# bifurcationkit/BifurcationKit.jl

Measured on NVIDIA H100. Metric: continuation steps/sec (SH2d PALC), higher is better.
Workload: dtype f64

## Files before the change

bifurcationkit.jl_b200/csrc/bk_async.cuh:

```cuda
#pragma once
#include "bk_common.cuh"

#ifdef __CUDACC__
__device__ __forceinline__ unsigned bk2_smem(const void* p) { return (unsigned)__cvta_generic_to_shared(p); }
__device__ __forceinline__ void mbar_init(unsigned long long* b, unsigned cnt) {
  asm volatile("mbarrier.init.shared::cta.b64 [%0], %1;" ::"r"(bk2_smem(b)), "r"(cnt) : "memory");
}
__device__ __forceinline__ void mbar_arrive_expect_tx(unsigned long long* b, unsigned bytes) {
  asm volatile("mbarrier.arrive.expect_tx.shared::cta.b64 _, [%0], %1;" ::"r"(bk2_smem(b)), "r"(bytes) : "memory");
}
__device__ __forceinline__ void mbar_arrive(unsigned long long* b) {
  asm volatile("mbarrier.arrive.shared::cta.b64 _, [%0];" ::"r"(bk2_smem(b)) : "memory");
}
__device__ __forceinline__ void mbar_wait(unsigned long long* b, unsigned parity) {
  asm volatile(
      "{\n"
      ".reg .pred p;\n"
      "BK2_WAIT_%=:\n"
      "mbarrier.try_wait.parity.shared::cta.b64 p, [%0], %1;\n"
      "@p bra BK2_DONE_%=;\n"
      "bra BK2_WAIT_%=;\n"
      "BK2_DONE_%=:\n"
      "}\n" ::"r"(bk2_smem(b)),
      "r"(parity)
      : "memory");
}
__device__ __forceinline__ void bulk_g2s(void* dst, const void* src, unsigned bytes, unsigned long long* bar) {
  asm volatile("cp.async.bulk.shared::cluster.global.mbarrier::complete_tx::bytes [%0], [%1], %2, [%3];" ::"r"(bk2_smem(dst)),
               "l"(src), "r"(bytes), "r"(bk2_smem(bar))
               : "memory");
}
__device__ __forceinline__ void bulk_s2g(void* dst, const void* src, unsigned bytes) {
  asm volatile("cp.async.bulk.global.shared::cta.bulk_group [%0], [%1], %2;" ::"l"(dst), "r"(bk2_smem(src)), "r"(bytes) : "memory");
}
__device__ __forceinline__ void bulk_store_commit() { asm volatile("cp.async.bulk.commit_group;" ::: "memory"); }
__device__ __forceinline__ void bulk_store_wait_read() { asm volatile("cp.async.bulk.wait_group.read 0;" ::: "memory"); }
__device__ __forceinline__ void bulk_store_wait_all() { asm volatile("cp.async.bulk.wait_group 0;" ::: "memory"); }
__device__ __forceinline__ void bulk_prefetch_l2(const void* src, unsigned bytes) {
  asm volatile("cp.async.bulk.prefetch.L2.global [%0], %1;" ::"l"(src), "r"(bytes) : "memory");
}
__device__ __forceinline__ void fence_proxy_async_smem() { asm volatile("fence.proxy.async.shared::cta;" ::: "memory"); }
#ifndef BK2_NO_WAR_FENCE
__device__ __forceinline__ void consumer_release_fence() { asm volatile("fence.proxy.async.shared::cta;" ::: "memory"); }
#else
__device__ __forceinline__ void consumer_release_fence() {}
#endif
__device__ __forceinline__ void fence_mbar_init() { asm volatile("fence.mbarrier_init.release.cluster;" ::: "memory"); }

#endif
```

bifurcationkit.jl_b200/csrc/bk_common.cuh:

```cuda
#pragma once
#include <cuda_runtime.h>
#include <stdint.h>
#include <stdlib.h>
#include <string>
#include <unordered_map>
#include <vector>
#include "../../include/bk200.h"
#include <nvtx3/nvToolsExt.h>

struct BkRange {
  explicit BkRange(const char* name) { nvtxRangePushA(name); }
  ~BkRange() { nvtxRangePop(); }
};

#define BK_MAX_PAR 8
#define BK_NSM_FALLBACK 132

struct OpDesc {
  int kind;
  int nx, ny, nz;
  double cx, cy, cz;
  double par[BK_MAX_PAR];
  const double* u;
  double a0, a1;
// ... 26 lines not shown
}

enum { PW_NONE = 0, PW_RESID = 1, PW_JVP = 2, PW_FLEFT = 3, PW_FRIGHT = 4 };
struct PerPw {
  int pro;
  int epi;
  const double* v;
  const double* u;
  const double* sp;
  double a0, a1, l, nu;
  double spc;
};
#define PW_D 1

struct Precond {
  int kind = BK_PC_NONE;
  double a0 = 0, a1 = 0;
  double* lam[3] = {nullptr, nullptr, nullptr};
  int ttype[3] = {0, 0, 0};
  int fast[3] = {0, 0, 0};
  double2* ftw[3] = {nullptr, nullptr, nullptr};
  double2* fom[3] = {nullptr, nullptr, nullptr};
  double2* flam2[3] = {nullptr, nullptr, nullptr};
  bkg::Plan gplan[3] = {};
  double2* gwl[3] = {nullptr, nullptr, nullptr};
  double2* gph[3] = {nullptr, nullptr, nullptr};
  double* work = nullptr;
  double* work2 = nullptr;
  double* tri = nullptr;
  double2* tdft = nullptr;
  double po_r = 0, po_nu = 0, po_T = 0;
};

struct BkKindTraits {
  int ndims;
  int fields;
  int extra;
  bool jac_sym;
  bool has_jt;
  bool complex_ok;
  bool pow2_grid;
  bool has_jets;
};
const BkKindTraits* bk_kind_traits(int kind);

struct BkEventTimer {
  std::vector<std::pair<cudaEvent_t, cudaEvent_t>> pairs;
  size_t used = 0;
  void begin(cudaStream_t st) {
    if (used == pairs.size()) {
      cudaEvent_t a, b;
      cudaEventCreate(&a);
      cudaEventCreate(&b);
      pairs.push_back({a, b});
    }
    cudaEventRecord(pairs[used++].first, st);
  }
  void end(cudaStream_t st) { cudaEventRecord(pairs[used - 1].second, st); }
  long long harvest(double& ms) {
    long long k = 0;
    for (size_t i = 0; i < used; ++i) {
      float t = 0;
      if (cudaEventElapsedTime(&t, pairs[i].first, pairs[i].second) == cudaSuccess) {
        ms += t;
        ++k;
      }
    }
    used = 0;
    return k;
  }
  void destroy() {
    for (auto& p : pairs) {
      cudaEventDestroy(p.first);
      cudaEventDestroy(p.second);
    }
    pairs.clear();
    used = 0;
  }
};

struct bk_ctx {
  int device = 0;
  int nsm = BK_NSM_FALLBACK;
  cudaStream_t stream = nullptr;
  int kind = 0;
  long long dims[3] = {1, 1, 1};
  double lengths[3] = {1, 1, 1};
  double par[BK_MAX_PAR] = {0};
  long long N = 0;
  long long N0 = 0;
  bool cplx = false;
  double shift_imag = 0;
  bool transpose = false;
  int m = 0;
  long long ld = 0;
  double* u_state = nullptr;
  double jpar[BK_MAX_PAR] = {0};
  bool have_state = false;
  double* phi = nullptr;
  double* xpi = nullptr;
  double* fcache = nullptr;
  double phi_dot_xpi = 0;
  double* V = nullptr;
  double* w = nullptr;
  double* z = nullptr;
  double* r = nullptr;
  double* scales = nullptr;
  double* gcoef = nullptr;
  double* hcols = nullptr;
  double* hcols2 = nullptr;
  double* h_pinned = nullptr;
  double* partials = nullptr;
  int gmax = 0;
  unsigned int* counters = nullptr;
  double* red_out = nullptr;
  double* red_pinned = nullptr;
  double* coef_pinned = nullptr;
  std::vector<cudaEvent_t> events;
  std::vector<double*> stage;
  double* host_pinned = nullptr;
  std::vector<double*> tmp;
  double* mom_stage = nullptr;
  size_t mom_stage_cap = 0;
  void* mom_work = nullptr;
  size_t mom_work_cap = 0;
  double* defl_pinned = nullptr;
  std::unordered_map<double*, size_t> vec_live;
  std::vector<std::pair<size_t, double*>> vec_pool;
  double* Q = nullptr;
  double* Q2 = nullptr;
  int q2cap = 0;
  int qcap = 0;
  double* eig_dev = nullptr;
  double* eig_pinned = nullptr;
  Precond pc;
  bk_stats stats = {};
  bool timing = false;
  int timing_every = 1;
  long long solve_count = 0;
  bool timing_now = false;
  BkEventTimer fused_timer;
  BkEventTimer pc_timer;
  std::unordered_map<const void*, size_t> smem_attr;
  std::string err;
};

int bk_fail(bk_ctx* c, int code, const char* what, const char* file, int line);
#define BK_CUDA(c, expr)                                                             \
  do {                                                                               \
    cudaError_t _e = (expr);                                                         \
    if (_e != cudaSuccess) return bk_fail((c), BK_ERR_CUDA, cudaGetErrorString(_e), __FILE__, __LINE__); \
  } while (0)
#define BK_CHECK(c, cond, msg)                                                       \
  do {                                                                               \
    if (!(cond)) return bk_fail((c), BK_ERR_ARG, (msg), __FILE__, __LINE__);         \
  } while (0)
#define BK_ENTER(c)                                 \
  do {                                              \
    if (!(c)) return BK_ERR_ARG;                    \
    if (cudaSetDevice((c)->device) != cudaSuccess)  \
      return bk_fail((c), BK_ERR_CUDA, "cudaSetDevice failed", __FILE__, __LINE__); \
  } while (0)
#define BK_TRY(expr)                 \
  do {                               \
    int _s = (expr);                 \
    if (_s < 0) return _s;           \
// ... 166 lines not shown
```

bifurcationkit.jl_b200/csrc/bk_ctx.cu:

```cuda
#include <cstdio>
#include <cstring>
#include <map>
#include <mutex>
#include <new>
#include "bk_common.cuh"

int bk_fail(bk_ctx* c, int code, const char* what, const char* file, int line) {
  if (c) {
    char buf[512];
    snprintf(buf, sizeof buf, "%s (%s:%d)", what, file, line);
    c->err = buf;
  }
  return code;
}

void bk_grant_smem(int device, const void* kern, size_t bytes) {
  static std::mutex mu;
  static std::map<std::pair<int, const void*>, size_t> granted;
  std::lock_guard<std::mutex> lk(mu);
  size_t& cur = granted[{device, kern}];
  if (bytes <= cur) return;
  cudaFuncSetAttribute(kern, cudaFuncAttributeMaxDynamicSharedMemorySize, (int)bytes);
  if (bytes > 48 * 1024) cudaFuncSetAttribute(kern, cudaFuncAttributePreferredSharedMemoryCarveout, 100);
  cur = bytes;
// ... 13 lines not shown
  BK_CHECK(c, p != nullptr, "null vector argument");
  if (bk_is_device_ptr(p)) {
    *dev = const_cast<double*>(p);
    return BK_OK;
  }
  BK_CHECK(c, slot >= 0 && slot < 16, "bad stage slot");
  if ((int)c->stage.size() <= slot) c->stage.resize(slot + 1, nullptr);
  if (!c->stage[slot]) BK_CUDA(c, cudaMalloc(&c->stage[slot], sizeof(double) * (size_t)c->ld));
  BK_CHECK(c, n <= c->ld, "vector longer than the context's leading dimension");
  if (copy_in) {
    BK_CUDA(c, cudaMemcpyAsync(c->stage[slot], p, sizeof(double) * (size_t)n, cudaMemcpyHostToDevice, c->stream));
    c->stats.h2d_bytes += 8 * n;
  }
  *dev = c->stage[slot];
  return BK_OK;
}

int bk_stage_out(bk_ctx* c, double* p, long long n, const double* dev) {
  if (p == dev) return BK_OK;
  BK_CUDA(c, cudaMemcpyAsync(p, dev, sizeof(double) * (size_t)n, cudaMemcpyDeviceToHost, c->stream));
  BK_CUDA(c, cudaStreamSynchronize(c->stream));
  c->stats.d2h_bytes += 8 * n;
  return BK_OK;
}

int bk_tmp(bk_ctx* c, int slot, double** out) {
  if ((int)c->tmp.size() <= slot) c->tmp.resize(slot + 1, nullptr);
  if (!c->tmp[slot]) BK_CUDA(c, cudaMalloc(&c->tmp[slot], sizeof(double) * (size_t)c->ld));
  *out = c->tmp[slot];
  return BK_OK;
}

const BkKindTraits* bk_kind_traits(int kind) {
  static const BkKindTraits table[] = {{0, 0, 0, false, false, false, false, false},
                                       {1, 1, 0, false, false, true, false, true},
                                       {2, 1, 0, true, true, true, false, true},
                                       {3, 1, 0, true, true, true, false, true},
                                       {2, 2, 0, false, true, true, false, true},
                                       {3, 2, 1, false, true, false, false, false},
                                       {2, 1, 0, true, true, true, true, true}};
  static_assert(BK_CHAN == 1 && BK_POTRAP_CGL2D == 5 && BK_SH2D_PERIODIC == 6, "the table is indexed by kind");
  if (kind < BK_CHAN || kind > BK_SH2D_PERIODIC) return nullptr;
  return &table[kind];
}

extern "C" int32_t bk_ctx_create(int32_t device, int32_t kind, const int64_t dims[3], const double lengths[3],
                                 int32_t krylov_m, bk_ctx** out) {
  if (!out) return BK_ERR_ARG;
  *out = nullptr;
  bk_ctx* c = new (std::nothrow) bk_ctx();
  if (!c) return BK_ERR_ARG;
  *out = c;
  c->device = device;
  c->cplx = (kind & BK_COMPLEX) != 0;
  kind &= ~BK_COMPLEX;
  c->kind = kind;
  for (int i = 0; i < 3; ++i) {
    c->dims[i] = dims ? (dims[i] > 0 ? dims[i] : 1) : 1;
    c->lengths[i] = lengths ? lengths[i] : 1.0;
  }
  const BkKindTraits* kt = bk_kind_traits(kind);
  if (!kt) return bk_fail(c, BK_ERR_ARG, "unknown problem kind", __FILE__, __LINE__);
  if (kt->pow2_grid)
    for (int d = 0; d < 2; ++d) {
      const long long v = c->dims[d];
      BK_CHECK(c, v >= 64 && v <= 2048 && (v & (v - 1)) == 0,
               "BK_SH2D_PERIODIC: Nx and Ny must be powers of two from 64 to 2048");
    }
  long long n = kt->fields;
  for (int d = 0; d < kt->ndims; ++d) n *= c->dims[d];
  n += kt->extra;
  BK_CHECK(c, n >= 2, "problem too small");
  BK_CHECK(c, krylov_m >= 1 && krylov_m <= 1024, "krylov_m out of range");
  BK_CHECK(c, !c->cplx || kt->complex_ok, "BK_COMPLEX is not available for the periodic-orbit functional");
  c->N0 = n;
  if (c->cplx) n *= 2;
  c->N = n;
  c->m = krylov_m;
  c->ld = ((n + 2 + 31) / 32) * 32;
  BK_CUDA(c, cudaSetDevice(device));
  cudaDeviceProp prop;
  BK_CUDA(c, cudaGetDeviceProperties(&prop, device));
  c->nsm = prop.multiProcessorCount;
  if (const char* e = getenv("BK_NSM")) {
    const int v = atoi(e);
    if (v >= 1 && v <= 1024) c->nsm = v;
  }
  BK_CUDA(c, cudaStreamCreateWithFlags(&c->stream, cudaStreamNonBlocking));
  size_t ld = (size_t)c->ld, m = (size_t)c->m;
  BK_CUDA(c, cudaMalloc(&c->u_state, 8 * ld));
  BK_CUDA(c, cudaMalloc(&c->V, 8 * ld * (m + 1)));
  BK_CUDA(c, cudaMalloc(&c->w, 8 * ld));
  BK_CUDA(c, cudaMalloc(&c->z, 8 * ld));
  BK_CUDA(c, cudaMalloc(&c->r, 8 * ld));
  BK_CUDA(c, cudaMemset(c->u_state, 0, 8 * ld));
  BK_CUDA(c, cudaMemset(c->V, 0, 8 * ld * (m + 1)));
  BK_CUDA(c, cudaMemset(c->w, 0, 8 * ld));
  BK_CUDA(c, cudaMemset(c->z, 0, 8 * ld));
  BK_CUDA(c, cudaMemset(c->r, 0, 8 * ld));
  BK_CUDA(c, cudaMalloc(&c->scales, 8 * (m + 4)));
  BK_CUDA(c, cudaMalloc(&c->gcoef, 8 * (m + 4)));
  BK_CUDA(c, cudaMalloc(&c->hcols, 8 * (m + 1) * (m + 4)));
  BK_CUDA(c, cudaMalloc(&c->hcols2, 8 * (m + 1) * (m + 4)));
  BK_CUDA(c, cudaMemset(c->hcols, 0, 8 * (m + 1) * (m + 4)));
  BK_CUDA(c, cudaMemset(c->hcols2, 0, 8 * (m + 1) * (m + 4)));
  BK_CUDA(c, cudaMallocHost(&c->h_pinned, 2 * 8 * (m + 1) * (m + 4)));
  long long g = (n + 2 + 255) / 256 + 8;
  if (kind == BK_SH2D) {
    long long gf = ((c->dims[0] + 255) / 256) * c->dims[1] + 8;
    if (gf > g) g = gf;
  }
  if (g < 4 * c->nsm) g = 4 * c->nsm;
  c->gmax = (int)g;
  BK_CUDA(c, cudaMalloc(&c->partials, 8 * (m + 4) * (size_t)c->gmax));
  BK_CUDA(c, cudaMalloc(&c->counters, 64 * sizeof(unsigned int)));
  BK_CUDA(c, cudaMemset(c->counters, 0, 64 * sizeof(unsigned int)));
  BK_CUDA(c, cudaMalloc(&c->red_out, 8 * 16));
  BK_CUDA(c, cudaMallocHost(&c->red_pinned, 8 * 16));
  BK_CUDA(c, cudaMallocHost(&c->coef_pinned, 8 * (m + 4)));
  c->events.resize(m + 2);
  for (auto& e : c->events) BK_CUDA(c, cudaEventCreateWithFlags(&e, cudaEventDisableTiming));
  if (kind == BK_POTRAP_CGL2D) {
    BK_CUDA(c, cudaMalloc(&c->phi, 8 * ld));
    BK_CUDA(c, cudaMalloc(&c->xpi, 8 * ld));
    BK_CUDA(c, cudaMalloc(&c->fcache, 8 * ld));
    BK_CUDA(c, cudaMemset(c->phi, 0, 8 * ld));
    BK_CUDA(c, cudaMemset(c->xpi, 0, 8 * ld));
  }
  if (kind == BK_SH2D_PERIODIC) BK_TRY(bk_periodic_setup(c));
  BK_CUDA(c, cudaStreamSynchronize(c->stream));
  return BK_OK;
}

extern "C" int32_t bk_ctx_destroy(bk_ctx* c) {
  if (!c) return BK_OK;
  cudaSetDevice(c->device);
  if (c->stream) cudaStreamSynchronize(c->stream);
  double* bufs[] = {c->u_state, c->V, c->w, c->z, c->r, c->scales, c->gcoef, c->hcols, c->hcols2, c->partials,
                    c->red_out, c->phi, c->xpi, c->fcache, c->pc.work, c->pc.work2, c->pc.tri, c->Q, c->Q2, c->eig_dev};
  for (double* b : bufs)
    if (b) cudaFree(b);
  for (int d = 0; d < 3; ++d) {
    void* tabs[] = {c->pc.lam[d], c->pc.ftw[d], c->pc.fom[d], c->pc.flam2[d], c->pc.gwl[d], c->pc.gph[d]};
    for (void* t : tabs)
      if (t) cudaFree(t);
  }
  if (c->pc.tdft) cudaFree(c->pc.tdft);
  if (c->counters) cudaFree(c->counters);
  for (auto& kv : c->vec_live) cudaFree(kv.first);
  for (double* b : c->stage)
    if (b) cudaFree(b);
  for (double* b : c->tmp)
    if (b) cudaFree(b);
  if (c->mom_stage) cudaFree(c->mom_stage);
  if (c->mom_work) cudaFree(c->mom_work);
  if (c->defl_pinned) cudaFreeHost(c->defl_pinned);
  if (c->h_pinned) cudaFreeHost(c->h_pinned);
  if (c->red_pinned) cudaFreeHost(c->red_pinned);
  if (c->coef_pinned) cudaFreeHost(c->coef_pinned);
  if (c->host_pinned) cudaFreeHost(c->host_pinned);
  if (c->eig_pinned) cudaFreeHost(c->eig_pinned);
  for (auto& e : c->events)
    if (e) cudaEventDestroy(e);
  c->fused_timer.destroy();
  c->pc_timer.destroy();
  if (c->stream) cudaStreamDestroy(c->stream);
// ... 214 lines not shown
```

bifurcationkit.jl_b200/csrc/bk_krylov.cu:

```cuda
#include <cmath>
#include <cstdlib>
#include <cstring>
#include <vector>
#include "bk_common.cuh"
#include "bk_stencil.cuh"
#include "bk_krylov_tma.cuh"

static __global__ void __launch_bounds__(BK_THREADS) k_lincomb(double* __restrict__ x, double beta, long long n,
                                                               const double* __restrict__ V, long long ld, int k,
                                                               const double* __restrict__ coef,
                                                               const double* __restrict__ scales) {
  const long long base = (long long)blockIdx.x * BK_TILE;
  double val[BK_EPT];
  int off[BK_EPT];
  bool ok[BK_EPT];
#pragma unroll
  for (int e = 0; e < BK_EPT; ++e) {
    long long g = base + threadIdx.x + e * BK_THREADS;
    ok[e] = g < n;
    off[e] = ok[e] ? (int)g : 0;
    val[e] = (ok[e] && beta != 0.0) ? beta * x[g] : 0.0;
  }
  for (int i = 0; i < k; ++i) {
    const double ci = coef[i] * (scales ? scales[i] : 1.0);
    const double* Vi = V + (long long)i * ld;
#pragma unroll
    for (int e = 0; e < BK_EPT; ++e) val[e] = fma(ci, __ldg(Vi + off[e]), val[e]);
  }
#pragma unroll
  for (int e = 0; e < BK_EPT; ++e)
    if (ok[e]) x[off[e]] = val[e];
}


#define BK2_BLOCKS_PER_SM 4
struct Plan2 {
  int E, grid, NS, sred_off;
  size_t smem;
};
static inline size_t bk2_budget() { return (size_t)(233472 / BK2_BLOCKS_PER_SM) - 1024 - 512; }

static Plan2 plan2(bk_ctx* c, long long units_of_256, size_t scratch_bytes_per_E(int), int force_E = 0) {
  Plan2 p;
  const long long slots = (long long)c->nsm * BK2_BLOCKS_PER_SM;
  long long E = BK2_EMAX;
  while (E > 1 && (units_of_256 + E - 1) / E < (17 * (long long)c->nsm) / 10) --E;
  if ((units_of_256 + E - 1) / E > slots) {
    double best = -1.0;
    for (long long cand = BK2_EMAX; cand >= 5; --cand) {
      long long g = (units_of_256 + cand - 1) / cand, w = (g + slots - 1) / slots;
      double eff = (double)g / (double)(w * slots);
      if (eff > best + 1e-9) {
        best = eff;
        E = cand;
      }
    }
  }
  if (force_E) E = force_E;
  {
    static const int env_e = [] {
      const char* a = getenv("BK2_E");
      return a ? atoi(a) : 0;
    }();
    if (env_e >= 1 && env_e <= BK2_EMAX) E = env_e;
  }
  p.E = (int)E;
  p.grid = (int)((units_of_256 + E - 1) / E);
  const size_t sred = sizeof(double) * 8 * (size_t)(c->m + 2);
  const size_t stage = sizeof(double) * (size_t)E * BK2_ROW;
  size_t budget = bk2_budget();
  long long ns = budget > sred ? (long long)((budget - sred) / stage) : 2;
  if (ns > BK2_MAXSTAGES) ns = BK2_MAXSTAGES;
  if (ns < 2) ns = 2;
  p.NS = (int)ns;
  size_t ring = stage * (size_t)p.NS;
  size_t scratch = scratch_bytes_per_E ? scratch_bytes_per_E(p.E) : 0;
  size_t lo = ring > scratch ? ring : scratch;
  lo = (lo + 127) / 128 * 128;
  p.sred_off = (int)(lo / sizeof(double));
  p.smem = lo + sred;
  return p;
}
static size_t sh2_scratch_bytes(int E) { return sizeof(double) * (size_t)((BK2_ROW + 4) * (E + 4) + (BK2_ROW + 2) * (E + 2)); }

#define BK2_DISPATCH(E, ...) \
  switch (E) {                \
    case 1: { constexpr int EE = 1; __VA_ARGS__; } break; \
    case 2: { constexpr int EE = 2; __VA_ARGS__; } break; \
    case 3: { constexpr int EE = 3; __VA_ARGS__; } break; \
    case 4: { constexpr int EE = 4; __VA_ARGS__; } break; \
    case 5: { constexpr int EE = 5; __VA_ARGS__; } break; \
    case 6: { constexpr int EE = 6; __VA_ARGS__; } break; \
    case 7: { constexpr int EE = 7; __VA_ARGS__; } break; \
    default: { constexpr int EE = 8; __VA_ARGS__; } break; \
  }

static bool fuses_jvp(const bk_ctx* c, const OpDesc& op, const bk_gmres_opts* o) {
  const bool left = o->pc_side == BK_SIDE_LEFT && c->pc.kind != BK_PC_NONE;
  return o->fused && op.kind == BK_SH2D && op.nx % 2 == 0 && !op.cplx && op.bordered <= 1 && !left;
}

static bool fuses_pc(const bk_ctx* c, const OpDesc& op, const bk_gmres_opts* o) {
  const bool side = o->pc_side == BK_SIDE_LEFT || o->pc_side == BK_SIDE_RIGHT;
  return o->fused && op.kind == BK_SH2D_PERIODIC && c->pc.kind == BK_PC_SH_FFT && side && op.bordered == 0 && !op.cplx;
}

static int launch_fused(bk_ctx* c, const OpDesc& op, const double* in, const double* sp, double* w, int j, double* hcol) {
  const int tiles_x = (op.nx + BK2_ROW - 1) / BK2_ROW;
  Plan2 p = plan2(c, (long long)tiles_x * op.ny, sh2_scratch_bytes);
  p.grid = tiles_x * ((op.ny + p.E - 1) / p.E);
  BK_CHECK(c, p.grid <= c->gmax, "partial-sum workspace too small for the fused grid");
  BK2_DISPATCH(p.E, {
    auto kern = op.bordered ? k2_fused<EE, true> : k2_fused<EE, false>;
    return bk_launch(c, kern, dim3(p.grid), dim3(BK2_THREADS), p.smem, op, in, sp, w, c->V, c->ld, j, c->scales, c->partials,
                     c->counters + 0, hcol, c->gcoef, p.NS, p.sred_off);
  });
}

static inline int chunk_grid(long long n) { return (int)((n + BK_TILE - 1) / BK_TILE); }

int bk_launch_dots(bk_ctx* c, const double* basis, const double* scales, const double* w, long long n, int j, double* hcol,
                   double* gcoef) {
  Plan2 p = plan2(c, (n + BK2_ROW - 1) / BK2_ROW, nullptr);
  BK_CHECK(c, p.grid <= c->gmax, "partial-sum workspace too small");
  BK2_DISPATCH(p.E, return bk_launch(c, k2_dots<EE>, dim3(p.grid), dim3(BK2_THREADS), p.smem, w, n, basis, c->ld, j, scales,
                                     c->partials, c->counters + 1, hcol, gcoef, p.NS, p.sred_off));
}
static int launch_dots(bk_ctx* c, const double* w, long long n, int j, double* hcol) {
  return bk_launch_dots(c, c->V, c->scales, w, n, j, hcol, c->gcoef);
}

int bk_launch_update(bk_ctx* c, const double* basis, const double* gcoef, const double* w, long long n, int j, double* vout,
                     double* h_out, double* scale_out) {
  Plan2 p = plan2(c, (n + BK2_ROW - 1) / BK2_ROW, nullptr);
  BK_CHECK(c, p.grid <= c->gmax, "partial-sum workspace too small");
  BK2_DISPATCH(p.E, return bk_launch(c, k2_update<EE>, dim3(p.grid), dim3(BK2_THREADS), p.smem, w, n, basis, c->ld, j, gcoef, vout,
                                     c->partials, c->counters + 2, h_out, scale_out, p.NS));
}
static int launch_update(bk_ctx* c, const double* w, long long n, int j, double* vout, double* h_out, double* scale_out) {
  return bk_launch_update(c, c->V, c->gcoef, w, n, j, vout, h_out, scale_out);
}

int bk_launch_lincomb(bk_ctx* c, const double* basis, const double* scales, double* x, double beta, long long n, int k,
                      const double* coef_dev) {
  return bk_launch_ordered(c, k_lincomb, chunk_grid(n), BK_THREADS, 0, x, beta, n, basis, c->ld, k, coef_dev, scales);
}
static int launch_lincomb(bk_ctx* c, double* x, double beta, long long n, int k, const double* coef_dev, bool use_scales) {
  return bk_launch_lincomb(c, c->V, use_scales ? c->scales : nullptr, x, beta, n, k, coef_dev);
}

static int arnoldi_step(bk_ctx* c, const OpDesc& op, const bk_gmres_opts* o, long long n, int k, bool fuse, bool fuse_pc) {
  const int j = k + 1;
  const int mh = c->m + 4;
  double* hcol = c->h_pinned + (size_t)k * mh;
  double* hcol2 = c->h_pinned + (size_t)(c->m + 1) * mh + (size_t)k * mh;
  const double* in = c->V + (size_t)k * c->ld;
  const double* sp = c->scales + k;
  const bool left = o->pc_side == BK_SIDE_LEFT && c->pc.kind != BK_PC_NONE;
  const bool right = o->pc_side == BK_SIDE_RIGHT && c->pc.kind != BK_PC_NONE;
  if (right && !fuse_pc) {
    BK_TRY(bk_precond_apply_dev(c, in, c->z, n));
    in = c->z;
  }
  const bool timed = c->timing_now;
  const double* wfin = c->w;
  if (fuse_pc) {
    BK_TRY(bk_periodic_fused(c, op, in, sp, c->w, left));
  } else if (!fuse) {
    BK_TRY(bk_launch_apply(c, op, in, sp, c->w));
    if (left) {
      BK_TRY(bk_precond_apply_dev(c, c->w, c->r, n));
      wfin = c->r;
    }
  }
  if (timed) c->fused_timer.begin(c->stream);
  BK_TRY(fuse ? launch_fused(c, op, in, sp, c->w, j, hcol) : launch_dots(c, wfin, n, j, hcol));
  if (timed) c->fused_timer.end(c->stream);
  double* vnext = c->V + (size_t)(k + 1) * c->ld;
  if (timed) c->fused_timer.begin(c->stream);
  BK_TRY(launch_update(c, wfin, n, j, vnext, hcol + j, c->scales + k + 1));
  if (timed) c->fused_timer.end(c->stream);
  if (o->orth == BK_ORTH_CGS2) {
    BK_TRY(launch_dots(c, vnext, n, j, hcol2));
    BK_TRY(launch_update(c, vnext, n, j, vnext, hcol + j, c->scales + k + 1));
  }
  BK_CUDA(c, cudaEventRecord(c->events[k], c->stream));
  const long long step_bytes = 8LL * n * (2LL * j + 4) + (op.bordered ? 16LL * n : 0LL);
  c->stats.last_fused_bytes += step_bytes;
  c->stats.last_fused_launches += 2;
  if (fuse && (c->timing_now || !c->timing)) {
    c->stats.total_fused_bytes += step_bytes;
    c->stats.total_fused_launches += 2;
  }
  return BK_OK;
}

static int init_residual(bk_ctx* c, const OpDesc& op, const bk_gmres_opts* o, long long n, const double* rhs, const double* x,
                         bool x_zero, double* beta) {
  const bool left = o->pc_side == BK_SIDE_LEFT && c->pc.kind != BK_PC_NONE;
  const double* r = rhs;
  if (!x_zero) {
    BK_TRY(bk_launch_apply(c, op, x, nullptr, c->w));
    BK_TRY(bk_dev_axpby(c, c->w, 1.0, rhs, -1.0, n));
    r = c->w;
  }
  if (left) {
    BK_TRY(bk_precond_apply_dev(c, r, c->r, n));
    r = c->r;
  }
  BK_TRY(launch_update(c, r, n, 0, c->V, c->red_out, c->scales));
  BK_CUDA(c, cudaMemcpyAsync(c->red_pinned, c->red_out, 8, cudaMemcpyDeviceToHost, c->stream));
  BK_CUDA(c, cudaStreamSynchronize(c->stream));
  *beta = c->red_pinned[0];
  return BK_OK;
}

int bk_gmres_dev(bk_ctx* c, const OpDesc& op, const double* rhs, double* x, const bk_gmres_opts* o, int* converged,
                 int* iters, double* resnorm) {
  const long long n = op.N + op.bordered;
  BK_CHECK(c, n <= c->ld, "system larger than the context");
// ... 183 lines not shown
```

bifurcationkit.jl_b200/csrc/bk_krylov_tma.cuh:

```cuda
#pragma once
#include "bk_common.cuh"
#include "bk_async.cuh"

#define BK2_CONS 256
#define BK2_THREADS 288
#define BK2_EMAX 8
#define BK2_ROW 256

struct Tile2 {
  long long base;
  int rs;
  int rows;
  int len;
  int last_len;
};

#define BK2_MAXSTAGES 8
struct Ring {
  unsigned long long full[BK2_MAXSTAGES];
  unsigned long long empty[BK2_MAXSTAGES];
};

__device__ __forceinline__ void ring_init(Ring* rg, int NS) {
  if (threadIdx.x == 0) {
    for (int s = 0; s < NS; ++s) {
      mbar_init(&rg->full[s], 1);
      mbar_init(&rg->empty[s], 8);
    }
    fence_mbar_init();
  }
}

template <int E, int MODE, bool REV = false>
__device__ __forceinline__ void stream_basis(const Tile2& tl, const double* __restrict__ V, long long ld, int j, double* ring,
                                             int NS, Ring* rg, double (&val)[E], double* sred,
                                             const double* __restrict__ gcoef) {
  const int warp = threadIdx.x >> 5, lane = threadIdx.x & 31;
  if (warp == 8) {
    if (lane == 0) {
      fence_proxy_async_smem();
      const unsigned row_b = (unsigned)(((tl.len + 1) & ~1) * 8);
      const unsigned last_b = (unsigned)(((tl.last_len + 1) & ~1) * 8);
      const bool contiguous = (tl.rs == BK2_ROW) && (tl.len == BK2_ROW);
      const unsigned total = row_b * (unsigned)(tl.rows - 1) + last_b;
      for (int i = 0; i < j; ++i) {
        const int s = i % NS, round = i / NS;
        if (round > 0) mbar_wait(&rg->empty[s], (unsigned)((round - 1) & 1));
        mbar_arrive_expect_tx(&rg->full[s], total);
        const double* src = V + (long long)(REV ? j - 1 - i : i) * ld + tl.base;
        double* dst = ring + (size_t)s * (E * BK2_ROW);
        if (contiguous) {
          bulk_g2s(dst, src, total, &rg->full[s]);
        } else {
          for (int r = 0; r < tl.rows - 1; ++r) bulk_g2s(dst + r * BK2_ROW, src + (long long)r * tl.rs, row_b, &rg->full[s]);
          bulk_g2s(dst + (tl.rows - 1) * BK2_ROW, src + (long long)(tl.rows - 1) * tl.rs, last_b, &rg->full[s]);
        }
      }
    }
  } else {
    const int t = threadIdx.x;
    if (MODE == 0) {
      for (int i = 0; i < j; i += 2) {
        const int s0 = i % NS, s1 = (i + 1) % NS;
        const bool two = (i + 1 < j);
        mbar_wait(&rg->full[s0], (unsigned)((i / NS) & 1));
        const double* st0 = ring + (size_t)s0 * (E * BK2_ROW) + t;
        double a0 = 0.0, a1 = 0.0;
#pragma unroll
        for (int e = 0; e < E; ++e) {
          const int lim = (e == tl.rows - 1) ? tl.last_len : tl.len;
          if (e < tl.rows && t < lim) a0 = fma(st0[e * BK2_ROW], val[e], a0);
        }
        if (two) {
          mbar_wait(&rg->full[s1], (unsigned)(((i + 1) / NS) & 1));
          const double* st1 = ring + (size_t)s1 * (E * BK2_ROW) + t;
#pragma unroll
          for (int e = 0; e < E; ++e) {
            const int lim = (e == tl.rows - 1) ? tl.last_len : tl.len;
            if (e < tl.rows && t < lim) a1 = fma(st1[e * BK2_ROW], val[e], a1);
          }
        }
        consumer_release_fence();
        __syncwarp();
        if (lane == 0) {
          mbar_arrive(&rg->empty[s0]);
          if (two) mbar_arrive(&rg->empty[s1]);
        }
#pragma unroll
        for (int o = 16; o > 0; o >>= 1) {
          a0 += __shfl_xor_sync(0xffffffffu, a0, o);
          a1 += __shfl_xor_sync(0xffffffffu, a1, o);
        }
        if (lane == 0) {
          sred[i * 8 + warp] = a0;
          if (two) sred[(i + 1) * 8 + warp] = a1;
        }
      }
    } else {
      for (int i = 0; i < j; ++i) {
        const int s = i % NS;
        mbar_wait(&rg->full[s], (unsigned)((i / NS) & 1));
        const double* st = ring + (size_t)s * (E * BK2_ROW) + t;
        const double g = __ldg(gcoef + (REV ? j - 1 - i : i));
#pragma unroll
        for (int e = 0; e < E; ++e) {
          const int lim = (e == tl.rows - 1) ? tl.last_len : tl.len;
          if (e < tl.rows && t < lim) val[e] = fma(-g, st[e * BK2_ROW], val[e]);
        }
        consumer_release_fence();
        __syncwarp();
        if (lane == 0) mbar_arrive(&rg->empty[s]);
      }
    }
  }
}

struct BorderFin {
  double bscale, bc, xp;
  double* w_tail;
  const double* V_tail;
  long long ld;
};
__device__ __forceinline__ void dots_finish(int j, const double* sred, const double* __restrict__ scales,
                                            double* __restrict__ partials, unsigned int* counter, double* __restrict__ hcol,
                                            double* __restrict__ gcoef, int* s_flag, const BorderFin* bord = nullptr,
                                            double* s_wp = nullptr) {
  const int G = gridDim.x;
  const int jj = bord ? j + 1 : j;
  for (int i = threadIdx.x; i < jj; i += blockDim.x) {
    double t = 0.0;
#pragma unroll
    for (int k = 0; k < 8; ++k) t += sred[i * 8 + k];
    partials[(long long)i * G + blockIdx.x] = t;
  }
  if (bk_last_block(counter, s_flag)) {
    const int warp = threadIdx.x >> 5, lane = threadIdx.x & 31, nw = blockDim.x >> 5;
    double wp = 0.0;
    if (bord) {
      if (warp == 0) {
        double t = 0.0;
        for (int k = lane; k < G; k += 32) t += __ldcg(partials + (long long)j * G + k);
        t = bk_warp_sum(t);
        if (lane == 0) {
          *s_wp = bord->bscale * t + bord->bc * bord->xp;
          *bord->w_tail = *s_wp;
        }
      }
      __syncthreads();
      wp = *s_wp;
    }
    for (int i = warp; i < j; i += nw) {
      double t = 0.0;
      for (int k = lane; k < G; k += 32) t += __ldcg(partials + (long long)i * G + k);
      t = bk_warp_sum(t);
      if (lane == 0) {
        if (bord) t = fma(__ldg(bord->V_tail + (long long)i * bord->ld), wp, t);
        const double s = scales[i];
        const double h = s * t;
        hcol[i] = h;
        gcoef[i] = h * s;
      }
    }
  }
}

template <int E>
struct Sh2Scratch {
  static constexpr int VX = BK2_ROW + 4, VY = E + 4, QX = BK2_ROW + 2, QY = E + 2;
  static constexpr int V_ELEMS = VX * VY, Q_ELEMS = QX * QY;
  static constexpr size_t BYTES = sizeof(double) * (size_t)(V_ELEMS + Q_ELEMS);
};

template <int E>
__device__ __forceinline__ void sh2_tile_issue(const OpDesc& op, const double* __restrict__ in, int x0, int y0, double* scratch,
                                               unsigned long long* tbar) {
  using S = Sh2Scratch<E>;
  const int nx = op.nx, ny = op.ny;
  const int len = min(BK2_ROW, nx - x0);
  mbar_arrive_expect_tx(tbar, (unsigned)(len * 8) * (unsigned)S::VY);
#pragma unroll 1
  for (int jj = 0; jj < S::VY; ++jj) {
    int gy = y0 - 2 + jj;
    gy = gy < 0 ? 0 : (gy > ny - 1 ? ny - 1 : gy);
    bulk_g2s(scratch + jj * S::VX + 2, in + x0 + (long long)gy * nx, (unsigned)(len * 8), tbar);
  }
}

template <int E, bool BORDERED, bool RESID = false>
__device__ __forceinline__ void sh2_tile_eval(const OpDesc& op, const double* __restrict__ in, double in_scale, int x0, int y0,
                                              double* scratch, unsigned long long* tbar, double (&val)[E], double xp,
                                              double* bsum) {
  using S = Sh2Scratch<E>;
  double* vs = scratch;
  double* qs = scratch + S::V_ELEMS;
  const int nx = op.nx, ny = op.ny;
  const int len = min(BK2_ROW, nx - x0);
  if (threadIdx.x < 4 * S::VY) {
    const int jj = threadIdx.x >> 2, h = threadIdx.x & 3;
    const int i = h < 2 ? h : len + h;
    int gx = x0 - 2 + i, gy = y0 - 2 + jj;
    gx = gx < 0 ? 0 : (gx > nx - 1 ? nx - 1 : gx);
    gy = gy < 0 ? 0 : (gy > ny - 1 ? ny - 1 : gy);
    vs[jj * S::VX + i] = __ldg(in + gx + (long long)gy * nx);
  }
  mbar_wait(tbar, 0);
  __syncthreads();
  for (int q = threadIdx.x; q < S::Q_ELEMS; q += blockDim.x) {
    int i = q % S::QX, jj = q / S::QX;
    int cx = x0 - 1 + i, cy = y0 - 1 + jj;
    cx = (cx < 0 ? 0 : (cx > nx - 1 ? nx - 1 : cx)) - (x0 - 2);
    cy = (cy < 0 ? 0 : (cy > ny - 1 ? ny - 1 : cy)) - (y0 - 2);
    const double* p = vs + cx + cy * S::VX;
    const double c0 = p[0];
    qs[q] = c0 + op.cx * (p[-1] - 2.0 * c0 + p[1]) + op.cy * (p[-S::VX] - 2.0 * c0 + p[S::VX]);
  }
  __syncthreads();
  const int t = threadIdx.x;
  const double l = op.par[0], nu = op.par[1];
  const int gx = x0 + t;
  const bool colok = t < BK2_ROW && gx < nx;
  const int rows = min(E, ny - y0);
  double g[E];
  if (!RESID) {
#pragma unroll
    for (int e = 0; e < E; ++e) g[e] = (colok && e < rows) ? __ldg(op.u + gx + (long long)(y0 + e) * nx) : 0.0;
  }
#pragma unroll
  for (int e = 0; e < E; ++e) {
    double r = 0.0;
    if (colok && e < rows) {
      const double* p = qs + (t + 1) + (e + 1) * S::QX;
      const double c0 = p[0];
      const double l1v = in_scale * (c0 + op.cx * (p[-1] - 2.0 * c0 + p[1]) + op.cy * (p[-S::QX] - 2.0 * c0 + p[S::QX]));
      const double v = in_scale * vs[(t + 2) + (e + 2) * S::VX];
      if (RESID) {
        r = v * (l + v * (nu - v)) - l1v;
      } else {
        const double coef = l + g[e] * (2.0 * nu - 3.0 * g[e]);
        r = op.a0 * v + op.a1 * (coef * v - l1v);
        if (BORDERED) r += op.bshift * v;
      }
    }
    val[e] = r;
  }
  if (BORDERED) {
#pragma unroll
    for (int e = 0; e < E; ++e) g[e] = (colok && e < rows) ? __ldg(op.ba + gx + (long long)(y0 + e) * nx) : 0.0;
#pragma unroll
    for (int e = 0; e < E; ++e) val[e] = fma(xp, g[e], val[e]);
#pragma unroll
    for (int e = 0; e < E; ++e) g[e] = (colok && e < rows) ? __ldg(op.bb + gx + (long long)(y0 + e) * nx) : 0.0;
#pragma unroll
    for (int e = 0; e < E; ++e)
      if (colok && e < rows) *bsum = fma(g[e], in_scale * vs[(t + 2) + (e + 2) * S::VX], *bsum);
  }
}

template <int E, bool BORDERED>
static __global__ void __launch_bounds__(BK2_THREADS, 4) k2_fused(OpDesc op, const double* __restrict__ in,
                                                                  const double* __restrict__ in_scale_ptr,
                                                                  double* __restrict__ w, const double* __restrict__ V,
                                                                  long long ld, int j, const double* __restrict__ scales,
                                                                  double* __restrict__ partials, unsigned int* counter,
                                                                  double* __restrict__ hcol, double* __restrict__ gcoef,
                                                                  int NS, int sred_off) {
  extern __shared__ __align__(128) double smem2[];
  __shared__ Ring rg;
  __shared__ __align__(8) unsigned long long tbar;
  __shared__ int s_flag;
  double* ring = smem2;
  double* sred = smem2 + sred_off;
  if (threadIdx.x == 0) mbar_init(&tbar, 1);
  ring_init(&rg, NS);
  const int tiles_x = (op.nx + BK2_ROW - 1) / BK2_ROW;
  const int x0 = (blockIdx.x % tiles_x) * BK2_ROW, y0 = (blockIdx.x / tiles_x) * E;
  double val[E];
  Tile2 tl;
  tl.base = x0 + (long long)y0 * op.nx;
  tl.rs = op.nx;
  tl.rows = min(E, op.ny - y0);
  tl.len = min(BK2_ROW, op.nx - x0);
  tl.last_len = tl.len;
  __syncthreads();
  bk_pdl_sync();
  const double s = in_scale_ptr ? __ldg(in_scale_ptr) : 1.0;
  if (threadIdx.x == BK2_CONS) {
    sh2_tile_issue<E>(op, in, x0, y0, smem2, &tbar);
    const unsigned row_b = (unsigned)(((tl.len + 1) & ~1) * 8);
    for (int r = 0; r < tl.rows; ++r) {
      const long long o = tl.base + (long long)r * tl.rs;
      bulk_prefetch_l2(op.u + o, row_b);
      if (BORDERED) {
        bulk_prefetch_l2(op.ba + o, row_b);
        bulk_prefetch_l2(op.bb + o, row_b);
      }
    }
    const int npf = j < 2 * NS ? j : 2 * NS;
    for (int i = 0; i < npf; ++i)
      for (int r = 0; r < tl.rows; ++r) bulk_prefetch_l2(V + (long long)i * ld + tl.base + (long long)r * tl.rs, row_b);
  }
  const double xp = BORDERED ? s * __ldg(in + op.N) : 0.0;
  double bsum = 0.0;
  sh2_tile_eval<E, BORDERED>(op, in, s, x0, y0, smem2, &tbar, val, xp, &bsum);
  if (threadIdx.x < tl.len) {
#pragma unroll
    for (int e = 0; e < E; ++e)
      if (e < tl.rows) w[tl.base + (long long)e * tl.rs + threadIdx.x] = val[e];
  }
  fence_proxy_async_smem();
  __syncthreads();
  stream_basis<E, 0>(tl, V, ld, j, ring, NS, &rg, val, sred, nullptr);
  if (BORDERED) {
    __shared__ double s_wp;
    bsum = bk_warp_sum(bsum);
    if ((threadIdx.x & 31) == 0 && threadIdx.x < BK2_CONS) sred[j * 8 + (threadIdx.x >> 5)] = bsum;
    __syncthreads();
    BorderFin bf;
    bf.bscale = op.bscale;
    bf.bc = op.bc;
    bf.xp = xp;
    bf.w_tail = w + op.N;
    bf.V_tail = V + op.N;
    bf.ld = ld;
    dots_finish(j, sred, scales, partials, counter, hcol, gcoef, &s_flag, &bf, &s_wp);
  } else {
    __syncthreads();
    dots_finish(j, sred, scales, partials, counter, hcol, gcoef, &s_flag);
  }
}

template <int E, int MODE>
static __global__ void __launch_bounds__(BK2_THREADS, 4) k2_apply(OpDesc op, const double* __restrict__ in,
                                                                  const double* __restrict__ in_scale_ptr, double* __restrict__ out) {
  extern __shared__ __align__(128) double smem2[];
  __shared__ __align__(8) unsigned long long tbar;
  if (threadIdx.x == 0) {
    mbar_init(&tbar, 1);
    fence_mbar_init();
  }
  const int tiles_x = (op.nx + BK2_ROW - 1) / BK2_ROW;
  const int x0 = (blockIdx.x % tiles_x) * BK2_ROW, y0 = (blockIdx.x / tiles_x) * E;
  const int rows = min(E, op.ny - y0), len = min(BK2_ROW, op.nx - x0);
  __syncthreads();
  const double s = in_scale_ptr ? __ldg(in_scale_ptr) : 1.0;
  if (threadIdx.x == BK2_CONS) {
    sh2_tile_issue<E>(op, in, x0, y0, smem2, &tbar);
    if (MODE == 0) {
      const unsigned row_b = (unsigned)(len * 8);
      for (int r = 0; r < rows; ++r) bulk_prefetch_l2(op.u + x0 + (long long)(y0 + r) * op.nx, row_b);
    }
  }
  double val[E];
  double bsum = 0.0;
  sh2_tile_eval<E, false, MODE == 1>(op, in, s, x0, y0, smem2, &tbar, val, 0.0, &bsum);
  if (threadIdx.x < len) {
#pragma unroll
    for (int e = 0; e < E; ++e)
      if (e < rows) out[x0 + (long long)(y0 + e) * op.nx + threadIdx.x] = val[e];
  }
}

__device__ __forceinline__ Tile2 linear_tile(long long n, int E) {
  Tile2 tl;
  tl.base = (long long)blockIdx.x * (E * BK2_ROW);
  tl.rs = BK2_ROW;
  long long rem = n - tl.base;
  int rows = (int)((rem + BK2_ROW - 1) / BK2_ROW);
  tl.rows = rows < E ? rows : E;
  tl.len = BK2_ROW;
  long long lastrem = rem - (long long)(tl.rows - 1) * BK2_ROW;
  tl.last_len = lastrem < BK2_ROW ? (int)lastrem : BK2_ROW;
  if (tl.rows == 1) tl.len = tl.last_len;
  return tl;
}

template <int E>
static __global__ void __launch_bounds__(BK2_THREADS, 4) k2_dots(const double* __restrict__ w, long long n,
                                                                 const double* __restrict__ V, long long ld, int j,
                                                                 const double* __restrict__ scales,
                                                                 double* __restrict__ partials, unsigned int* counter,
                                                                 double* __restrict__ hcol, double* __restrict__ gcoef, int NS,
                                                                 int sred_off) {
  extern __shared__ __align__(128) double smem2[];
  __shared__ Ring rg;
  __shared__ int s_flag;
  double* ring = smem2;
  double* sred = smem2 + sred_off;
  ring_init(&rg, NS);
  const Tile2 tl = linear_tile(n, E);
  double val[E];
  bk_pdl_sync();
#pragma unroll
  for (int e = 0; e < E; ++e) {
    const int lim = (e == tl.rows - 1) ? tl.last_len : tl.len;
    val[e] = (threadIdx.x < BK2_ROW && e < tl.rows && (int)threadIdx.x < lim) ? w[tl.base + e * BK2_ROW + threadIdx.x] : 0.0;
  }
  __syncthreads();
  stream_basis<E, 0>(tl, V, ld, j, ring, NS, &rg, val, sred, nullptr);
  __syncthreads();
  dots_finish(j, sred, scales, partials, counter, hcol, gcoef, &s_flag);
}

template <int E>
static __global__ void __launch_bounds__(BK2_THREADS, 4) k2_update(const double* w, long long n,
                                                                   const double* __restrict__ V, long long ld, int j,
                                                                   const double* __restrict__ gcoef, double* vout,
                                                                   double* __restrict__ partials, unsigned int* counter,
                                                                   double* __restrict__ h_out, double* __restrict__ scale_out,
                                                                   int NS) {
  extern __shared__ __align__(128) double smem2[];
  __shared__ Ring rg;
  __shared__ double s_w[9];
  __shared__ int s_flag;
  double* ring = smem2;
  ring_init(&rg, NS);
  const Tile2 tl = linear_tile(n, E);
  double val[E];
  const int t = threadIdx.x;
  bk_pdl_sync();
#pragma unroll
  for (int e = 0; e < E; ++e) {
    const int lim = (e == tl.rows - 1) ? tl.last_len : tl.len;
    val[e] = (t < BK2_ROW && e < tl.rows && t < lim) ? w[tl.base + e * BK2_ROW + t] : 0.0;
  }
  __syncthreads();
  stream_basis<E, 1, true>(tl, V, ld, j, ring, NS, &rg, val, nullptr, gcoef);
  double acc = 0.0;
  if (t < BK2_ROW) {
#pragma unroll
    for (int e = 0; e < E; ++e) {
      const int lim = (e == tl.rows - 1) ? tl.last_len : tl.len;
      if (e < tl.rows && t < lim) {
        vout[tl.base + e * BK2_ROW + t] = val[e];
        acc = fma(val[e], val[e], acc);
      }
    }
  }
  acc = bk_warp_sum(acc);
  const int lane = t & 31, wid = t >> 5;
  if (lane == 0) s_w[wid] = acc;
  __syncthreads();
  if (t == 0) {
    double r = 0;
    for (int k = 0; k < 9; ++k) r += s_w[k];
    partials[blockIdx.x] = r;
  }
  if (bk_last_block(counter, &s_flag)) {
    double r = 0.0;
    for (int k = t; k < (int)gridDim.x; k += blockDim.x) r += __ldcg(partials + k);
    r = bk_warp_sum(r);
    if (lane == 0) s_w[wid] = r;
    __syncthreads();
    if (t == 0) {
      double q = 0;
      for (int k = 0; k < 9; ++k) q += s_w[k];
      const double h = sqrt(q);
      *h_out = h;
      *scale_out = 1.0 / h;
    }
  }
}
```

Before: 4.343.

## Add L2 evict-first/evict-last hints to Krylov basis streaming and reorder fused kernel

Krylov basis loads through the bulk-copy ring now carry an L2 cache policy. The last `keep` vectors, sized to about half the L2, are marked evict-last so they stay resident for the next kernel; older ones are marked evict-first. The explicit L2 prefetch of the first basis vectors in the fused kernel is removed. The stencil kernel issues its state loads before the halo barrier, and the fused kernel writes w after streaming the basis rather than before. The aim is fewer DRAM re-reads of recently used basis vectors and more overlap of latency, at the risk of mis-sized keep windows and of losing the prefetch's head start.

```diff
diff --git a/bifurcationkit.jl_b200/csrc/bk_async.cuh b/bifurcationkit.jl_b200/csrc/bk_async.cuh
--- a/bifurcationkit.jl_b200/csrc/bk_async.cuh
+++ b/bifurcationkit.jl_b200/csrc/bk_async.cuh
@@ -30,6 +30,24 @@
                "l"(src), "r"(bytes), "r"(bk2_smem(bar))
                : "memory");
 }
+__device__ __forceinline__ unsigned long long l2_evict_first() {
+  unsigned long long p;
+  asm volatile("createpolicy.fractional.L2::evict_first.b64 %0, 1.0;" : "=l"(p));
+  return p;
+}
+__device__ __forceinline__ unsigned long long l2_evict_last() {
+  unsigned long long p;
+  asm volatile("createpolicy.fractional.L2::evict_last.b64 %0, 1.0;" : "=l"(p));
+  return p;
+}
+__device__ __forceinline__ void bulk_g2s(void* dst, const void* src, unsigned bytes, unsigned long long* bar,
+                                         unsigned long long policy) {
+  asm volatile(
+      "cp.async.bulk.shared::cluster.global.mbarrier::complete_tx::bytes.L2::cache_hint [%0], [%1], %2, [%3], %4;" ::"r"(
+          bk2_smem(dst)),
+      "l"(src), "r"(bytes), "r"(bk2_smem(bar)), "l"(policy)
+      : "memory");
+}
 __device__ __forceinline__ void bulk_s2g(void* dst, const void* src, unsigned bytes) {
   asm volatile("cp.async.bulk.global.shared::cta.bulk_group [%0], [%1], %2;" ::"l"(dst), "r"(bk2_smem(src)), "r"(bytes) : "memory");
 }
diff --git a/bifurcationkit.jl_b200/csrc/bk_common.cuh b/bifurcationkit.jl_b200/csrc/bk_common.cuh
--- a/bifurcationkit.jl_b200/csrc/bk_common.cuh
+++ b/bifurcationkit.jl_b200/csrc/bk_common.cuh
@@ -132,6 +132,7 @@
 struct bk_ctx {
   int device = 0;
   int nsm = BK_NSM_FALLBACK;
+  long long l2_bytes = 0;
   cudaStream_t stream = nullptr;
   int kind = 0;
   long long dims[3] = {1, 1, 1};
diff --git a/bifurcationkit.jl_b200/csrc/bk_ctx.cu b/bifurcationkit.jl_b200/csrc/bk_ctx.cu
--- a/bifurcationkit.jl_b200/csrc/bk_ctx.cu
+++ b/bifurcationkit.jl_b200/csrc/bk_ctx.cu
@@ -119,6 +119,7 @@
   cudaDeviceProp prop;
   BK_CUDA(c, cudaGetDeviceProperties(&prop, device));
   c->nsm = prop.multiProcessorCount;
+  c->l2_bytes = prop.l2CacheSize;
   if (const char* e = getenv("BK_NSM")) {
     const int v = atoi(e);
     if (v >= 1 && v <= 1024) c->nsm = v;
diff --git a/bifurcationkit.jl_b200/csrc/bk_krylov.cu b/bifurcationkit.jl_b200/csrc/bk_krylov.cu
--- a/bifurcationkit.jl_b200/csrc/bk_krylov.cu
+++ b/bifurcationkit.jl_b200/csrc/bk_krylov.cu
@@ -35,7 +35,7 @@
 
 #define BK2_BLOCKS_PER_SM 4
 struct Plan2 {
-  int E, grid, NS, sred_off;
+  int E, grid, NS, sred_off, keep;
   size_t smem;
 };
 static inline size_t bk2_budget() { return (size_t)(233472 / BK2_BLOCKS_PER_SM) - 1024 - 512; }
@@ -79,6 +79,7 @@
   lo = (lo + 127) / 128 * 128;
   p.sred_off = (int)(lo / sizeof(double));
   p.smem = lo + sred;
+  p.keep = (int)(c->l2_bytes / 2 / (units_of_256 * BK2_ROW * (long long)sizeof(double)));
   return p;
 }
 static size_t sh2_scratch_bytes(int E) { return sizeof(double) * (size_t)((BK2_ROW + 4) * (E + 4) + (BK2_ROW + 2) * (E + 2)); }
@@ -113,7 +114,7 @@
   BK2_DISPATCH(p.E, {
     auto kern = op.bordered ? k2_fused<EE, true> : k2_fused<EE, false>;
     return bk_launch(c, kern, dim3(p.grid), dim3(BK2_THREADS), p.smem, op, in, sp, w, c->V, c->ld, j, c->scales, c->partials,
-                     c->counters + 0, hcol, c->gcoef, p.NS, p.sred_off);
+                     c->counters + 0, hcol, c->gcoef, p.keep, p.NS, p.sred_off);
   });
 }
 
@@ -124,7 +125,7 @@
   Plan2 p = plan2(c, (n + BK2_ROW - 1) / BK2_ROW, nullptr);
   BK_CHECK(c, p.grid <= c->gmax, "partial-sum workspace too small");
   BK2_DISPATCH(p.E, return bk_launch(c, k2_dots<EE>, dim3(p.grid), dim3(BK2_THREADS), p.smem, w, n, basis, c->ld, j, scales,
-                                     c->partials, c->counters + 1, hcol, gcoef, p.NS, p.sred_off));
+                                     c->partials, c->counters + 1, hcol, gcoef, p.keep, p.NS, p.sred_off));
 }
 static int launch_dots(bk_ctx* c, const double* w, long long n, int j, double* hcol) {
   return bk_launch_dots(c, c->V, c->scales, w, n, j, hcol, c->gcoef);
@@ -135,7 +136,7 @@
   Plan2 p = plan2(c, (n + BK2_ROW - 1) / BK2_ROW, nullptr);
   BK_CHECK(c, p.grid <= c->gmax, "partial-sum workspace too small");
   BK2_DISPATCH(p.E, return bk_launch(c, k2_update<EE>, dim3(p.grid), dim3(BK2_THREADS), p.smem, w, n, basis, c->ld, j, gcoef, vout,
-                                     c->partials, c->counters + 2, h_out, scale_out, p.NS));
+                                     c->partials, c->counters + 2, h_out, scale_out, p.keep, p.NS));
 }
 static int launch_update(bk_ctx* c, const double* w, long long n, int j, double* vout, double* h_out, double* scale_out) {
   return bk_launch_update(c, c->V, c->gcoef, w, n, j, vout, h_out, scale_out);
diff --git a/bifurcationkit.jl_b200/csrc/bk_krylov_tma.cuh b/bifurcationkit.jl_b200/csrc/bk_krylov_tma.cuh
--- a/bifurcationkit.jl_b200/csrc/bk_krylov_tma.cuh
+++ b/bifurcationkit.jl_b200/csrc/bk_krylov_tma.cuh
@@ -32,8 +32,8 @@
 }
 
 template <int E, int MODE, bool REV = false>
-__device__ __forceinline__ void stream_basis(const Tile2& tl, const double* __restrict__ V, long long ld, int j, double* ring,
-                                             int NS, Ring* rg, double (&val)[E], double* sred,
+__device__ __forceinline__ void stream_basis(const Tile2& tl, const double* __restrict__ V, long long ld, int j, int keep,
+                                             double* ring, int NS, Ring* rg, double (&val)[E], double* sred,
                                              const double* __restrict__ gcoef) {
   const int warp = threadIdx.x >> 5, lane = threadIdx.x & 31;
   if (warp == 8) {
@@ -43,17 +43,20 @@
       const unsigned last_b = (unsigned)(((tl.last_len + 1) & ~1) * 8);
       const bool contiguous = (tl.rs == BK2_ROW) && (tl.len == BK2_ROW);
       const unsigned total = row_b * (unsigned)(tl.rows - 1) + last_b;
+      const unsigned long long pol_first = l2_evict_first(), pol_last = l2_evict_last();
       for (int i = 0; i < j; ++i) {
         const int s = i % NS, round = i / NS;
         if (round > 0) mbar_wait(&rg->empty[s], (unsigned)((round - 1) & 1));
         mbar_arrive_expect_tx(&rg->full[s], total);
         const double* src = V + (long long)(REV ? j - 1 - i : i) * ld + tl.base;
         double* dst = ring + (size_t)s * (E * BK2_ROW);
+        const unsigned long long pol = i >= j - keep ? pol_last : pol_first;
         if (contiguous) {
-          bulk_g2s(dst, src, total, &rg->full[s]);
+          bulk_g2s(dst, src, total, &rg->full[s], pol);
         } else {
-          for (int r = 0; r < tl.rows - 1; ++r) bulk_g2s(dst + r * BK2_ROW, src + (long long)r * tl.rs, row_b, &rg->full[s]);
-          bulk_g2s(dst + (tl.rows - 1) * BK2_ROW, src + (long long)(tl.rows - 1) * tl.rs, last_b, &rg->full[s]);
+          for (int r = 0; r < tl.rows - 1; ++r)
+            bulk_g2s(dst + r * BK2_ROW, src + (long long)r * tl.rs, row_b, &rg->full[s], pol);
+          bulk_g2s(dst + (tl.rows - 1) * BK2_ROW, src + (long long)(tl.rows - 1) * tl.rs, last_b, &rg->full[s], pol);
         }
       }
     }
@@ -195,6 +198,16 @@
   double* qs = scratch + S::V_ELEMS;
   const int nx = op.nx, ny = op.ny;
   const int len = min(BK2_ROW, nx - x0);
+  const int t = threadIdx.x;
+  const double l = op.par[0], nu = op.par[1];
+  const int gx = x0 + t;
+  const bool colok = t < BK2_ROW && gx < nx;
+  const int rows = min(E, ny - y0);
+  double g[E];
+  if (!RESID) {
+#pragma unroll
+    for (int e = 0; e < E; ++e) g[e] = (colok && e < rows) ? __ldg(op.u + gx + (long long)(y0 + e) * nx) : 0.0;
+  }
   if (threadIdx.x < 4 * S::VY) {
     const int jj = threadIdx.x >> 2, h = threadIdx.x & 3;
     const int i = h < 2 ? h : len + h;
@@ -215,16 +228,6 @@
     qs[q] = c0 + op.cx * (p[-1] - 2.0 * c0 + p[1]) + op.cy * (p[-S::VX] - 2.0 * c0 + p[S::VX]);
   }
   __syncthreads();
-  const int t = threadIdx.x;
-  const double l = op.par[0], nu = op.par[1];
-  const int gx = x0 + t;
-  const bool colok = t < BK2_ROW && gx < nx;
-  const int rows = min(E, ny - y0);
-  double g[E];
-  if (!RESID) {
-#pragma unroll
-    for (int e = 0; e < E; ++e) g[e] = (colok && e < rows) ? __ldg(op.u + gx + (long long)(y0 + e) * nx) : 0.0;
-  }
 #pragma unroll
   for (int e = 0; e < E; ++e) {
     double r = 0.0;
@@ -263,7 +266,7 @@
                                                                   long long ld, int j, const double* __restrict__ scales,
                                                                   double* __restrict__ partials, unsigned int* counter,
                                                                   double* __restrict__ hcol, double* __restrict__ gcoef,
-                                                                  int NS, int sred_off) {
+                                                                  int keep, int NS, int sred_off) {
   extern __shared__ __align__(128) double smem2[];
   __shared__ Ring rg;
   __shared__ __align__(8) unsigned long long tbar;
@@ -295,21 +298,18 @@
         bulk_prefetch_l2(op.bb + o, row_b);
       }
     }
-    const int npf = j < 2 * NS ? j : 2 * NS;
-    for (int i = 0; i < npf; ++i)
-      for (int r = 0; r < tl.rows; ++r) bulk_prefetch_l2(V + (long long)i * ld + tl.base + (long long)r * tl.rs, row_b);
   }
   const double xp = BORDERED ? s * __ldg(in + op.N) : 0.0;
   double bsum = 0.0;
   sh2_tile_eval<E, BORDERED>(op, in, s, x0, y0, smem2, &tbar, val, xp, &bsum);
+  fence_proxy_async_smem();
+  __syncthreads();
+  stream_basis<E, 0>(tl, V, ld, j, keep, ring, NS, &rg, val, sred, nullptr);
   if (threadIdx.x < tl.len) {
 #pragma unroll
     for (int e = 0; e < E; ++e)
       if (e < tl.rows) w[tl.base + (long long)e * tl.rs + threadIdx.x] = val[e];
   }
-  fence_proxy_async_smem();
-  __syncthreads();
-  stream_basis<E, 0>(tl, V, ld, j, ring, NS, &rg, val, sred, nullptr);
   if (BORDERED) {
     __shared__ double s_wp;
     bsum = bk_warp_sum(bsum);
@@ -379,8 +379,8 @@
                                                                  const double* __restrict__ V, long long ld, int j,
                                                                  const double* __restrict__ scales,
                                                                  double* __restrict__ partials, unsigned int* counter,
-                                                                 double* __restrict__ hcol, double* __restrict__ gcoef, int NS,
-                                                                 int sred_off) {
+                                                                 double* __restrict__ hcol, double* __restrict__ gcoef, int keep,
+                                                                 int NS, int sred_off) {
   extern __shared__ __align__(128) double smem2[];
   __shared__ Ring rg;
   __shared__ int s_flag;
@@ -396,7 +396,7 @@
     val[e] = (threadIdx.x < BK2_ROW && e < tl.rows && (int)threadIdx.x < lim) ? w[tl.base + e * BK2_ROW + threadIdx.x] : 0.0;
   }
   __syncthreads();
-  stream_basis<E, 0>(tl, V, ld, j, ring, NS, &rg, val, sred, nullptr);
+  stream_basis<E, 0>(tl, V, ld, j, keep, ring, NS, &rg, val, sred, nullptr);
   __syncthreads();
   dots_finish(j, sred, scales, partials, counter, hcol, gcoef, &s_flag);
 }
@@ -407,7 +407,7 @@
                                                                    const double* __restrict__ gcoef, double* vout,
                                                                    double* __restrict__ partials, unsigned int* counter,
                                                                    double* __restrict__ h_out, double* __restrict__ scale_out,
-                                                                   int NS) {
+                                                                   int keep, int NS) {
   extern __shared__ __align__(128) double smem2[];
   __shared__ Ring rg;
   __shared__ double s_w[9];
@@ -424,7 +424,7 @@
     val[e] = (t < BK2_ROW && e < tl.rows && t < lim) ? w[tl.base + e * BK2_ROW + t] : 0.0;
   }
   __syncthreads();
-  stream_basis<E, 1, true>(tl, V, ld, j, ring, NS, &rg, val, nullptr, gcoef);
+  stream_basis<E, 1, true>(tl, V, ld, j, keep, ring, NS, &rg, val, nullptr, gcoef);
   double acc = 0.0;
   if (t < BK2_ROW) {
 #pragma unroll
```

After: 4.496, median of 6. +3.5%, better.
